# LabJunBMI/E3-invaraint-diffusion-model

Hardware: AMD Instinct MI355X
Metric: denoising-steps/sec (batched pocket graphs) (higher is better)
Workload: dtype f32 storage and accumulation, f16x3 products (fp32 grade); 1 GPU; structure_model sampling step, 256 x 256-residue pockets per GPU, 12+12 layers x 768, T=1000 schedule, encoder recomputed every step (as the reference); pockets_per_gpu=256, seq_len=256, parallelism=pocket-sharded x1, no collective

## Files before the change

e3-invaraint-diffusion-model_amd/bert.py:

```python
from dataclasses import dataclass

import os

import torch
from torch import nn

from . import ops
from .autograd import functional as F


@dataclass
class BertConfig:
    hidden_size: int = 768
    num_attention_heads: int = 12
    intermediate_size: int = 1024
    num_hidden_layers: int = 12
    max_position_embeddings: int = 64
    position_embedding_type: str = "relative_key"
    hidden_dropout_prob: float = 0.1
    attention_probs_dropout_prob: float = 0.1
    layer_norm_eps: float = 1e-12
    hidden_act: str = "gelu"
    use_cache: bool = False
    is_decoder: bool = False
# ... 172 lines not shown
def run_self_attention(att, x, mask, B, L, drop=(0.0, 0.0), layout=None):
    sa = att.self
    w, b = qkv_weights(sa)
    qkv = F.linear(x, w, b, absmax=ops.absmax_slot(sa, "qkv", x.device))
    relkey = sa.position_embedding_type == "relative_key"
    if layout is not None:
        H = att.num_heads * 64
        ctx = ops.attention_varlen(qkv[:, :H], qkv[:, H:2 * H], qkv[:, 2 * H:], layout, layout, att.num_heads,
                                   dist_emb=sa.distance_embedding.weight if relkey else None,
                                   max_pos=sa.max_position_embeddings)
        return _attention_output(att, ctx, x)
    ctx = F.attention(qkv, None, B, att.num_heads, L, L, key_mask=mask,
                      dist_emb=sa.distance_embedding.weight if relkey else None,
                      max_pos=sa.max_position_embeddings, drop_p=drop[1], row_keys=drop_keys(drop),
                      planes_for=_planes_for(att, x, drop))
    return _attention_output(att, ctx, x, drop[0], drop_keys(drop))


def project_cross_kv(att, enc):
    w, b = kv_weights(att.self)
    return F.linear(enc, w, b, absmax=torch.zeros(1, device=enc.device, dtype=torch.float32))


def run_cross_attention(att, x, kv, enc_mask, B, Lq, Lk, drop=(0.0, 0.0), layout=None, enc_layout=None):
    q = F.linear(x, att.self.query.weight, att.self.query.bias, absmax=ops.absmax_slot(att.self, "q", x.device))
    if layout is not None:
        H = att.num_heads * 64
        ctx = ops.attention_varlen(q, kv[:, :H], kv[:, H:], layout, enc_layout, att.num_heads)
        return _attention_output(att, ctx, x)
    ctx = F.attention(q, kv, B, att.num_heads, Lq, Lk, key_mask=enc_mask, drop_p=drop[1], row_keys=drop_keys(drop),
                      planes_for=_planes_for(att, x, drop))
    return _attention_output(att, ctx, x, drop[0], drop_keys(drop))


def run_layer(layer, x, mask, B, L, cross_kv=None, enc_mask=None, Lk=None, drop=(0.0, 0.0), layout=None,
              enc_layout=None):
    x = run_self_attention(layer.attention, x, mask, B, L, drop, layout=layout)
    if hasattr(layer, "crossattention"):
        if cross_kv is None:
            raise ValueError("decoder layer needs encoder states")
        x = run_cross_attention(layer.crossattention, x, cross_kv, enc_mask, B, L, Lk, drop, layout=layout,
                                enc_layout=enc_layout)
    inter = F.linear(x, layer.intermediate.dense.weight, layer.intermediate.dense.bias, ops.ACT_GELU,
                     planes_for=(layer.output.dense.weight, x) if drop[0] == 0 and drop[1] == 0 else None)
    return F.linear_residual_layernorm(inter, layer.output.dense.weight, layer.output.dense.bias, x,
                                       layer.output.LayerNorm.weight, layer.output.LayerNorm.bias, layer.eps, drop[0],
# ... 17 lines not shown
```

e3-invaraint-diffusion-model_amd/csrc/gemm_split.hip:

```cpp
#include <type_traits>

#include "e3d_common.h"

namespace {

typedef __bf16 bf16x8 __attribute__((ext_vector_type(8)));
typedef __bf16 bf16x4 __attribute__((ext_vector_type(4)));
typedef _Float16 f16x8 __attribute__((ext_vector_type(8)));
typedef _Float16 f16x4 __attribute__((ext_vector_type(4)));

template <typename E> struct Vec;
template <> struct Vec<__bf16> { typedef bf16x8 x8; typedef bf16x4 x4; };
template <> struct Vec<_Float16> { typedef f16x8 x8; typedef f16x4 x4; };
__device__ __forceinline__ f32x16 mma16(const bf16x8 a, const bf16x8 b, const f32x16 c) {
    return __builtin_amdgcn_mfma_f32_32x32x16_bf16(a, b, c, 0, 0, 0);
}
__device__ __forceinline__ f32x16 mma16(const f16x8 a, const f16x8 b, const f32x16 c) {
    return __builtin_amdgcn_mfma_f32_32x32x16_f16(a, b, c, 0, 0, 0);
}

struct Epi { float* absmax; float scale; int plan_m = 0; const int* run_if = nullptr; };

constexpr int BN = 128, BK = 32;
#ifdef GEMM_STAMPS
// ... 689 lines not shown
            const int col = col0 + wc * 64 + n * 32 + l31;
            const float bv = bias ? bias[col] : 0.f;
#pragma unroll
            for (int r = 0; r < 16; ++r) {
                const int row = row0 + wr * 128 + m * 32 + mfma32_row(r, half);
                float v = fmaf(acc[m][n][r], out_scale, bv);
                if (ACT == E3D_ACT_GELU) v = gelu_erf(v);
                if (ACT == E3D_ACT_SILU) v = silu(v);
                if (row < M) {
                    out[(int64_t)row * ldc + col] = v;
                    if (ACT == E3D_ACT_NONE && absmax) e3d_absmax_accum(amax, v);
                }
            }
        }
    }
    if (ACT == E3D_ACT_NONE && absmax) e3d_absmax_commit(amax, absmax, lane);
    STAMP_K(4);
#ifdef E3D_STAMPS
    asm volatile("s_waitcnt vmcnt(0)" ::: "memory");
    STAMP_K(5);
#endif
}

#ifdef E3D_NT_STORES
#define E3D_STORE_OUT(ptr, val) __builtin_nontemporal_store((val), (ptr))
#else
#define E3D_STORE_OUT(ptr, val) (*(ptr) = (val))
#endif

template <int ACT, typename E, bool PLANES = false>
__global__ __launch_bounds__(512, 2) void gemm_split256p_kernel(const float* __restrict__ A, int64_t lda,
                                                                 const float* __restrict__ W,
                                                                 const float* __restrict__ bias,
                                                                 float* __restrict__ out, int64_t ldc, int N, int K,
                                                                 int tiles_m, int tiles_n, float* __restrict__ absmax, float out_scale,
                                                                 const int* __restrict__ run_if) {
    if (run_if && *run_if == 0) return;
    extern __shared__ __attribute__((aligned(16))) unsigned char smem_raw[];
    constexpr int NS = 2, T_BYTES = BT * ROW64, BUF_BYTES = 2 * NS * T_BYTES;
    constexpr int NI = 8;
    const int total = tiles_m * tiles_n, nk = K / BK;
    const int tid = threadIdx.x, lane = tid & 63, wid = tid >> 6;
    const int wr = wid >> 2, wc = wid & 3;
    const int l31 = lane & 31, half = lane >> 5;

    unsigned goff[NI];
    int dst[NI];
#pragma unroll
    for (int i = 0; i < NI; ++i) {
        const int f = tid + 512 * (i & 3), r = f >> 3, kg = f & 7;
        goff[i] = (unsigned)(r * (i < 4 ? (int)lda : K) + kg * 4);
        dst[i] = (i < 4 ? 0 : NS * T_BYTES) + swz_off(r, kg >> 1) + (kg & 1) * 8;
    }

    int ld_tile = blockIdx.x, ld_k = 0;
    const float* ld_a;
    const float* ld_w;
    auto cursor_bases = [&]() {
        const int lid = xcd_remap(ld_tile, total);
        ld_a = A + (int64_t)(lid / tiles_n) * BT * lda + ld_k * BK;
        ld_w = W + (int64_t)(lid % tiles_n) * BT * K + ld_k * BK;
    };
    auto cursor_advance = [&]() {
        if (ld_k + 1 < nk) {
            ++ld_k;
            ld_a += BK;
            ld_w += BK;
        } else if (ld_tile + (int)gridDim.x < total) {
            ld_tile += gridDim.x;
            ld_k = 0;
            cursor_bases();
        }
    };
    f32x4 rg[NI];
    auto item_load = [&](int i) { rg[i] = *reinterpret_cast<const f32x4*>((i < 4 ? ld_a : ld_w) + goff[i]); };
    auto item_store = [&](int i, unsigned char* buf) {
        typename Vec<E>::x4 p[NS];
        split4<NS, E>(rg[i], p);
#pragma unroll
        for (int s = 0; s < NS; ++s) *reinterpret_cast<typename Vec<E>::x4*>(buf + s * T_BYTES + dst[i]) = p[s];
    };
    cursor_bases();
#pragma unroll
    for (int i = 0; i < NI; ++i) item_load(i);
    cursor_advance();
#pragma unroll
    for (int i = 0; i < NI; ++i) item_store(i, smem_raw);
#pragma unroll
    for (int i = 0; i < NI; ++i) item_load(i);
    cursor_advance();
    __syncthreads();

    int a_row[4], b_row[2];
#pragma unroll
    for (int m = 0; m < 4; ++m) a_row[m] = wr * 128 + m * 32 + l31;
#pragma unroll
    for (int n = 0; n < 2; ++n) b_row[n] = wc * 64 + n * 32 + l31;
    int cur = 0;
    unsigned amax = 0;

    for (int tile = blockIdx.x; tile < total; tile += gridDim.x) {
        f32x16 acc[4][2];
#pragma unroll
        for (int m = 0; m < 4; ++m)
#pragma unroll
            for (int n = 0; n < 2; ++n)
#pragma unroll
                for (int r = 0; r < 16; ++r) acc[m][n][r] = 0.f;
        for (int kt = 0; kt < nk; ++kt) {
            const unsigned char* base = smem_raw + cur * BUF_BYTES;
            unsigned char* next = smem_raw + (cur ^ 1) * BUF_BYTES;
#pragma unroll
            for (int ks = 0; ks < 2; ++ks) {
                typename Vec<E>::x8 fa[NS][4], fb[NS][2];
#pragma unroll
                for (int s = 0; s < NS; ++s) {
#pragma unroll
                    for (int n = 0; n < 2; ++n)
                        fb[s][n] = *reinterpret_cast<const typename Vec<E>::x8*>(base + (NS + s) * T_BYTES +
                                                                    swz_off(b_row[n], 2 * ks + half));
#pragma unroll
                    for (int m = 0; m < 4; ++m)
// ... 55 lines not shown
                        for (int j = 0; j < 4; ++j) {
                            float a = fmaf(acc[m][n][8 * kl + j], out_scale, bl[8 * kl + j]);
                            float c = fmaf(acc[m][n][8 * kl + 4 + j], out_scale, bl[8 * kl + 4 + j]);
                            if (ACT == E3D_ACT_GELU) { a = gelu_erf(a); c = gelu_erf(c); }
                            if (ACT == E3D_ACT_SILU) { a = silu(a); c = silu(c); }
                            if (ACT == E3D_ACT_NONE && absmax) { e3d_absmax_accum(amax, a); e3d_absmax_accum(amax, c); }
                            asm volatile("" : "+v"(a));
                            asm volatile("" : "+v"(c));
                            const auto sw = __builtin_amdgcn_permlane32_swap(__float_as_uint(a), __float_as_uint(c), false, false);
                            x0[j] = __uint_as_float(sw[0]);
                            x1[j] = __uint_as_float(sw[1]);
                        }
                        typename Vec<E>::x4 p0[2], p1[2];
                        split4<2, E>(x0, p0);
                        split4<2, E>(x1, p1);
                        typedef typename Vec<E>::x8 X8;
                        *reinterpret_cast<X8*>(o + kl * 2048) = __builtin_shufflevector(p0[0], p1[0], 0, 1, 2, 3, 4, 5, 6, 7);
                        *reinterpret_cast<X8*>(o + kl * 2048 + 1024) = __builtin_shufflevector(p0[1], p1[1], 0, 1, 2, 3, 4, 5, 6, 7);
                    }
                }
            }
            continue;
        }
        const int lid = xcd_remap(tile, total);
        const int row0 = (lid / tiles_n) * BT, col0 = (lid % tiles_n) * BT;
#pragma unroll
        for (int m = 0; m < 4; ++m) {
#pragma unroll
            for (int n = 0; n < 2; ++n) {
                const int col = col0 + wc * 64 + n * 32 + l31;
                const float bv = bias ? bias[col] : 0.f;
                float* o = out + (int64_t)(row0 + wr * 128 + m * 32 + 4 * half) * ldc + col;
#pragma unroll
                for (int r = 0; r < 16; ++r) {
                    float v = fmaf(acc[m][n][r], out_scale, bv);
                    if (ACT == E3D_ACT_GELU) v = gelu_erf(v);
                    if (ACT == E3D_ACT_SILU) v = silu(v);
                    E3D_STORE_OUT(&o[(int64_t)((r & 3) + 8 * (r >> 2)) * ldc], v);
                    if (ACT == E3D_ACT_NONE && absmax) e3d_absmax_accum(amax, v);
                }
            }
        }
    }
    if (ACT == E3D_ACT_NONE && absmax) e3d_absmax_commit(amax, absmax, lane);
}

template <int ACT, typename E, bool PLANES = false>
int launch256p(const float* A, int64_t lda, const float* W, const float* bias, float* out, int64_t ldc, int M, int N,
               int K, Epi epi, hipStream_t s) {
    const int tiles_m = M / BT, tiles_n = N / BT;
    constexpr size_t lds = 2 * 2 * 2 * BT * ROW64;
    static std::atomic<uint64_t> lds_ok{0};
    const int n_cu = e3d_cu_count();
    const int total = tiles_m * tiles_n;
    e3d_allow_lds(lds_ok, gemm_split256p_kernel<ACT, E, PLANES>, lds);
    hipLaunchKernelGGL((gemm_split256p_kernel<ACT, E, PLANES>), dim3(total < n_cu ? total : n_cu), dim3(512), lds, s, A, lda, W, bias, out,
                       ldc, N, K, tiles_m, tiles_n, epi.absmax, epi.scale, epi.run_if);
    return e3d_launch_status(PLANES ? "e3d_gemm_bias_act_planes_split (persistent 256x256)" : "e3d_gemm_f32_split (persistent 256x256)");
}

int g_general_form = -1;
int g_tile_pref = -1;

template <int NS, int ACT, int WR, int WC, int NBUF, bool PIPE, typename E>
int launch256(const float* A, int64_t lda, const float* W, const float* bias, float* out, int64_t ldc, int M, int N,
              int K, Epi epi, hipStream_t s) {
    constexpr int TM = WR * 128, TN = WC * 64;
    const int tiles_m = (M + TM - 1) / TM, tiles_n = N / TN;
    const size_t lds = (size_t)NBUF * NS * (TM + TN) * ROW64;
    static std::atomic<uint64_t> lds_ok{0};
    e3d_allow_lds(lds_ok, gemm_split256_kernel<NS, ACT, WR, WC, NBUF, PIPE, E>, lds);
    hipLaunchKernelGGL((gemm_split256_kernel<NS, ACT, WR, WC, NBUF, PIPE, E>), dim3(tiles_m * tiles_n), dim3(WR * WC * 64), lds, s,
                       A, lda, W, bias, out, ldc, M, N, K, tiles_m, tiles_n, epi.absmax, epi.scale, epi.run_if);
    return e3d_launch_status("e3d_gemm_f32_split (128x64 wave tiles)");
}

template <int NS, int ACT, bool A_KMAJ, bool B_KMAJ, int WM, int WN, typename E, int TN = 2, bool TR = false>
int launch_general(const float* A, int64_t lda, const float* B, int64_t ldb, const float* bias, float* out, int64_t ldc,
                   int M, int N, int K, Epi epi, hipStream_t s);

int p_min() {
    static int v = 0;
    if (!v) {
        const char* e = getenv("E3D_GEMM_P_MIN");
        v = e ? atoi(e) : 160;
    }
    return v;
}

bool persistent_ok(int M, int Mp, int N, int K, int64_t lda, int64_t ldb, int k_min = 2 * BK) {
    if (g_tile_pref < 0) {
        const char* e = getenv("E3D_GEMM_TILE");
        g_tile_pref = e ? atoi(e) : 4;
    }
    const int64_t n_tiles = (int64_t)(Mp / BT) * (N / BT);
    return N % BT == 0 && M % BT == 0 && Mp % BT == 0 && ldb == K && g_tile_pref >= 4 && K >= k_min && lda < (1 << 22) &&
           (g_tile_pref >= 5 || n_tiles >= p_min() || (n_tiles >= 96 && N >= 6 * BT && !getenv("E3D_GEMM_P_MIN")));
}

template <int NS, int ACT, bool A_KMAJ, bool B_KMAJ, typename E>
int launch(const float* A, int64_t lda, const float* B, int64_t ldb, const float* bias, float* out, int64_t ldc,
           int M, int N, int K, Epi epi, hipStream_t s) {
    if (g_tile_pref < 0) {
        const char* e = getenv("E3D_GEMM_TILE");
        g_tile_pref = e ? atoi(e) : 4;
    }
    const int Mp = epi.plan_m > 0 ? epi.plan_m : M;
    if constexpr (!A_KMAJ && !B_KMAJ) {
        if constexpr (NS == 2) {
            if (persistent_ok(M, Mp, N, K, lda, ldb))
                return launch256p<ACT, E>(A, lda, B, bias, out, ldc, M, N, K, epi, s);
            if (N % BT == 0 && ldb == K && g_tile_pref >= 3 && (int64_t)((Mp + BT - 1) / BT) * (N / BT) >= 256)
                return launch256<NS, ACT, 2, 4, 2, true, E>(A, lda, B, bias, out, ldc, M, N, K, epi, s);
        }
        if constexpr (NS == 1) {
            if (N % BT == 0 && ldb == K && g_tile_pref >= 3 && (int64_t)((Mp + BT - 1) / BT) * (N / BT) >= 160)
                return launch256<NS, ACT, 2, 4, 2, true, E>(A, lda, B, bias, out, ldc, M, N, K, epi, s);
        }
        if (N % BT == 0 && ldb == K && g_tile_pref >= 1 &&
            (int64_t)((Mp + BT - 1) / BT) * (N / BT) >= 256)
            return launch256<NS, ACT, 2, 4, (NS <= 2 ? 2 : 1), false, E>(A, lda, B, bias, out, ldc, M, N, K, epi, s);
    }
    if (g_general_form < 0) {
        const char* e = getenv("E3D_GEMM_FORM");
        g_general_form = e ? atoi(e) : 0;
    }
    int form = g_general_form;
    if (form != 1 && form != 2 && form != 3 && form != 4) {
        const int64_t g256 = (int64_t)((Mp + 255) / 256) * ((N + 127) / 128), g128 = (int64_t)((Mp + 127) / 128) * ((N + 127) / 128);
        const int64_t cus = e3d_cu_count();
        if (NS == 3) form = g256 < 128 && !A_KMAJ && !B_KMAJ ? 2 : 1;
        else if (A_KMAJ && B_KMAJ) form = 1;
        else if (A_KMAJ) form = g128 <= cus ? 2 : (g256 <= cus ? 1 : (45 * ((g128 + 2 * cus - 1) / (2 * cus)) < 37 * ((g256 + cus - 1) / cus) ? 2 : 1));
        else form = 25 * ((g128 + cus - 1) / cus) <= 38 * ((g256 + cus - 1) / cus) ? 3 : 1;
// ... 76 lines not shown
    if (a_kmaj && b_kmaj) return launch<NS, E3D_ACT_NONE, true, true, __bf16>(A, lda, B, ldb, bias, out, ldc, M, N, K, Epi{nullptr, epi.scale}, s);
    return launch<NS, E3D_ACT_NONE, true, false, __bf16>(A, lda, B, ldb, bias, out, ldc, M, N, K, epi, s);
}

}

#ifdef GEMM_STAMPS
extern "C" int e3d_debug_gemm_stamps(long long* t) { return (int)hipMemcpyFromSymbol(t, HIP_SYMBOL(gemm_stamps), sizeof(long long) * 2 * 64 * 8); }
#endif

#ifdef E3D_STAMPS
extern "C" int e3d_debug_read_stamps(long long* host_out) {
    return (int)hipMemcpyFromSymbol(host_out, HIP_SYMBOL(e3d_stamps), sizeof(long long) * 2 * 32 * 8);
}
#endif

extern "C" int e3d_gemm_kernel_select(int pref) {
    if (g_tile_pref < 0) {
        const char* e = getenv("E3D_GEMM_TILE");
        g_tile_pref = e ? atoi(e) : 4;
    }
    const int prev = g_tile_pref;
    if (pref >= 0) g_tile_pref = pref;
    return prev;
}

extern "C" int e3d_gemm_general_select(int form) {
    if (g_general_form < 0) {
        const char* e = getenv("E3D_GEMM_FORM");
        g_general_form = e ? atoi(e) : 0;
    }
    const int prev = g_general_form;
    if (form >= 0) g_general_form = form;
    return prev;
}

static int gemm_split_general(const float* A, int64_t lda, int a_kmajor, const float* B, int64_t ldb, int b_kmajor,
                              const float* bias, float* out, int64_t ldc, int M, int N, int K, int act, int terms,
                              float* absmax, float out_scale, void* stream, int plan_m = 0, const int* run_if = nullptr) {
    const Epi epi{absmax, out_scale, plan_m, run_if};
    E3D_REQUIRE(plan_m >= 0 && (!(a_kmajor || b_kmajor) || (plan_m == 0 && !run_if)),
                "gemm_split: plan_m / run_if exist for the forward (K-contiguous) layout (plan_m=%d)", plan_m);
    E3D_REQUIRE(out_scale == 1.0f || !(a_kmajor && b_kmajor), "gemm_split: out_scale is not available for the split-K layout");
    E3D_REQUIRE(A && B && out, "gemm_split: null pointer");
    E3D_REQUIRE(M > 0 && N > 0 && K > 0, "gemm_split: bad shape M=%d N=%d K=%d", M, N, K);
    E3D_REQUIRE(terms == E3D_TERMS_BF16 || terms == 3 || terms == 6 || terms == E3D_TERMS_F16X3,
// ... 145 lines not shown
    return (terms == 3 || terms == E3D_TERMS_F16X3) && (act == E3D_ACT_NONE || act == E3D_ACT_GELU) && M > 0 && N > 0 && K > 0 &&
           K % BK == 0 && lda >= K && lda % 4 == 0 && persistent_ok(M, M, N, K, lda, K, BK);
}

extern "C" int e3d_gemm_bias_act_planes_split(const float* A, int64_t lda, const float* W, const float* bias, void* out_planes,
                                              int M, int N, int K, int act, int terms, float* out_absmax, float out_scale,
                                              void* stream) {
    E3D_REQUIRE(A && W && out_planes, "gemm_split (planes): null pointer");
    E3D_REQUIRE(e3d_gemm_planes_supported(M, N, K, lda, act, terms),
                "gemm_split (planes): this launch does not take the persistent kernel (M=%d N=%d K=%d act=%d terms=%d)", M, N, K, act, terms);
    E3D_REQUIRE(((uintptr_t)A % 16) == 0 && ((uintptr_t)W % 16) == 0 && ((uintptr_t)bias % 16) == 0 && ((uintptr_t)out_planes % 16) == 0,
                "gemm_split (planes): A, W, bias and the planes must be 16-byte aligned");
    E3D_REQUIRE(!out_absmax || act == E3D_ACT_NONE, "gemm_split (planes): out_absmax exists for act = none");
    const Epi epi{out_absmax, out_scale, 0, nullptr};
    hipStream_t s = (hipStream_t)stream;
    float* out = reinterpret_cast<float*>(out_planes);
    if (terms == 3) {
        if (act == E3D_ACT_GELU) return launch256p<E3D_ACT_GELU, __bf16, true>(A, lda, W, bias, out, N, M, N, K, epi, s);
        return launch256p<E3D_ACT_NONE, __bf16, true>(A, lda, W, bias, out, N, M, N, K, epi, s);
    }
    if (act == E3D_ACT_GELU) return launch256p<E3D_ACT_GELU, _Float16, true>(A, lda, W, bias, out, N, M, N, K, epi, s);
    return launch256p<E3D_ACT_NONE, _Float16, true>(A, lda, W, bias, out, N, M, N, K, epi, s);
}
```

e3-invaraint-diffusion-model_amd/hip.py:

```python
import ctypes
import os
from ctypes import c_char_p, c_float, c_int, c_int64, c_uint32, c_uint64, c_void_p

_HERE = os.path.dirname(os.path.abspath(__file__))
LIB_PATH = os.environ.get("E3D_HIP_LIB", os.path.join(_HERE, "libe3d_hip.so"))
ABI_VERSION = 5

_P = c_void_p
_VIEW = [_P, c_int64, c_int64]
_QKV = 3 * _VIEW + [_P, c_int, _P]
_SHAPE = 4 * [c_int]
_ATTN_FWD = _QKV + [_P, _P] + _SHAPE
_ATTN_BWD = _QKV + 3 * [_P] + 3 * _VIEW + [_P, _P] + _SHAPE
_STREAM = [_P]
_DROP = [c_float, c_uint64]
_DROP_KEYED = [c_float, c_uint32, _P]
_BOUNDS = [_P, c_int, _P, _P, _P]
_SIGNATURES = {
    "e3d_abi_version": (c_int, []),
    "e3d_last_error": (c_char_p, []),
    "e3d_gemm_bias_act_f32": (c_int, [_P, c_int64, _P, _P, _P, c_int64, c_int, c_int, c_int, c_int, _P]),
    "e3d_gemm_bias_act_f32_split": (c_int, [_P, c_int64, _P, _P, _P, c_int64, c_int, c_int, c_int, c_int, c_int, _P]),
    "e3d_gemm_bias_act_f32_split_ex": (c_int, [_P, c_int64, _P, _P, _P, c_int64, c_int, c_int, c_int, c_int, c_int, _P, c_float, _P]),
    "e3d_gemm_bias_act_f32_split_gated": (c_int, [_P, c_int64, _P, _P, _P, c_int64, c_int, c_int, c_int, c_int, c_int, _P, c_float,
                                                  c_int, _P, _P]),
    "e3d_absmax_f32": (c_int, [_P, c_int64, _P, _P]),
    "e3d_relkey_attn_fwd": (c_int, _ATTN_FWD + _STREAM),
    "e3d_relkey_attn_fwd_split": (c_int, _ATTN_FWD + [c_int] + _STREAM),
    "e3d_gemm_skinny_workspace_bytes": (c_int64, [c_int, c_int, c_int]),
    "e3d_gemm_skinny_f32_split": (c_int, [_P, c_int64, _P, _P, _P, c_int64, c_int, c_int, c_int, c_int, c_int, _P, c_int64, _P]),
    "e3d_gemm_skinny_f32_split_ex": (c_int, [_P, c_int64, _P, _P, _P, c_int64, c_int, c_int, c_int, c_int, c_int, _P, c_int64, _P, c_float, _P]),
    "e3d_gemm_skinny_plan_select": (None, [c_int, c_int]),
    "e3d_gemm_skinny_residual_layernorm_f32_split": (c_int, [_P, c_int64, _P, _P, _P, _P, _P, c_float, _P, c_int, c_int, c_int,
                                                     c_int, _P, c_int64, _P]),
    "e3d_gemm_skinny_residual_layernorm_f32_split_ex": (c_int, [_P, c_int64, _P, _P, _P, _P, _P, c_float, _P, c_int, c_int, c_int,
                                                        c_int, _P, c_int64, c_float, _P]),
    "e3d_attn_skip_padded_tiles": (c_int, [c_int]),
    "e3d_gemm_kernel_select": (c_int, [c_int]),
    "e3d_gemm_general_select": (c_int, [c_int]),
    "e3d_attn_rescale_tau": (c_float, [c_float]),
    "e3d_residual_layernorm_fwd": (c_int, [_P, _P, _P, _P, c_float, _P, _P, c_int, c_int, _P]),
    "e3d_adaln_gate_fwd": (c_int, [_P, _P, _P, c_int, c_int, _P, c_int, c_int, _P]),
    "e3d_embed_layernorm_fwd": (c_int, [_P, c_int, _P, _P, _P, _P, c_float, _P, c_int, _P, _P, c_int, c_int, _P]),
    "e3d_adaln_gate_indexed_fwd": (c_int, [_P, _P, _P, _P, c_int, _P, c_int, _P, c_int, c_int, _P]),
    "e3d_classify_onehot_rows": (c_int, [_P, c_int, _P, _P, c_int, _P]),
    "e3d_embed_layernorm_fwd_ex": (c_int, [_P, c_int, _P, _P, _P, _P, c_float, _P, c_int, _P, _P, c_int, c_int, _P, _P]),
    "e3d_nerf_backbone": (c_int, [_P, _P, _P, c_int, c_int, c_int, _P]),
    "e3d_gemm_f32_split_general": (c_int, [_P, c_int64, c_int, _P, c_int64, c_int, _P, _P, c_int64, c_int, c_int,
                                           c_int, c_int, c_int, _P]),
    "e3d_transpose_grouped_f32": (c_int, [_P, _P, c_int, c_int, c_int, c_int64, c_int64, _P]),
    "e3d_gemm_wgrad_grouped_f32_split": (c_int, [_P, _P, _P, _P, c_uint64, c_int, c_int64, c_int64, c_int, c_int, c_int, c_int, _P]),
    "e3d_residual_layernorm_drop_fwd": (c_int, [_P, _P, _P, _P, c_float, _P, _P, c_int, c_int, c_float, c_uint64, _P]),
    "e3d_layernorm_bwd_drop": (c_int, [_P, _P, _P, c_float, _P, _P, _P, _P, c_int, c_int, c_float, c_uint64, _P]),
    "e3d_weight_planes_bytes": (c_int64, [c_int, c_int]),
    "e3d_weight_planes_f32_split": (c_int, [_P, c_int, c_int, c_int, _P, _P]),
    "e3d_gemm_residual_layernorm_supported": (c_int, [c_int, c_int, c_int, c_int64]),
    "e3d_gemm_residual_layernorm_f32_split": (c_int, [_P, c_int64, _P, _P, _P, c_int64, _P, _P, c_float, _P, c_int64,
                                                      c_int, c_int, c_int, c_int, c_float, _P]),
    "e3d_activation_planes_bytes": (c_int64, [c_int, c_int]),
    "e3d_activation_planes_f32_split": (c_int, [_P, c_int64, c_int, c_int, c_int, _P, _P]),
    "e3d_gemm_residual_layernorm_planes_split": (c_int, [_P, _P, _P, _P, c_int64, _P, _P, c_float, _P, c_int64,
                                                         c_int, c_int, c_int, c_int, c_float, _P]),
    "e3d_gemm_planes_supported": (c_int, [c_int, c_int, c_int, c_int64, c_int, c_int]),
    "e3d_gemm_bias_act_planes_split": (c_int, [_P, c_int64, _P, _P, _P, c_int, c_int, c_int, c_int, c_int, _P, c_float, _P]),
    "e3d_attn_planes_supported": (c_int, [c_int64, c_int64, c_int64, c_int, c_int, c_int, c_int]),
    "e3d_relkey_attn_fwd_split_planes": (c_int, _QKV + [_P] + _SHAPE + [c_int] + _BOUNDS + _STREAM),
    "e3d_gemm_wgrad_ragged_f32_split": (c_int, [_P, _P, _P, _P, _P, _P, _P, _P, c_uint64, c_int, c_int, c_int, _P]),
    "e3d_relkey_attn_bwd_workspace_floats": (c_int64, [c_int, c_int, c_int, c_int, c_int]),
    "e3d_relkey_attn_bwd": (c_int, _ATTN_BWD + _STREAM),
    "e3d_dropout_f32": (c_int, [_P, c_float, c_uint64, _P, c_int64, _P]),
    "e3d_relkey_attn_fwd_split_drop": (c_int, _ATTN_FWD + [c_int] + _DROP + _STREAM),
    "e3d_relkey_attn_fwd_split_ex": (c_int, _ATTN_FWD + [c_int] + _DROP + _BOUNDS + _STREAM),
    "e3d_attn_scratch_bytes": (c_int64, [c_int]),
    "e3d_ddpm_step_wrap_table": (c_int, [_P, _P, _P, _P, _P, c_int, _P, c_int64, _P]),
    "e3d_relkey_attn_bwd_drop": (c_int, _ATTN_BWD + _DROP + _STREAM),
    "e3d_relkey_attn_bwd_ex": (c_int, _ATTN_BWD + [c_int] + _DROP + _STREAM),
    "e3d_attn_dropout_mask": (c_int, [c_int, c_int, c_int, c_int, c_float, c_uint64, _P, _P]),
    "e3d_layernorm_bwd": (c_int, [_P, _P, _P, c_float, _P, _P, _P, c_int, c_int, _P]),
    "e3d_layernorm_bwd_workspace_floats": (c_int64, [c_int, c_int]),
    "e3d_layernorm_bwd_ws": (c_int, [_P, _P, _P, c_float, _P, _P, _P, _P, c_int, c_int, c_float, c_uint64, _P, c_int64, _P]),
    "e3d_adaln_gate_bwd": (c_int, [_P, _P, _P, c_int, c_int, _P, _P, c_int, c_int, _P]),
    "e3d_act_fwd": (c_int, [_P, c_int, _P, c_int64, _P]),
    "e3d_act_bwd": (c_int, [_P, _P, c_int, _P, c_int64, _P]),
    "e3d_colsum": (c_int, [_P, c_int64, _P, c_int, c_int, _P]),
    "e3d_group_sum": (c_int, [_P, c_int, _P, c_int, c_int, _P]),
    "e3d_small_k_wgrad": (c_int, [_P, _P, _P, _P, c_int, c_int, c_int, c_int, _P]),
    "e3d_head_linear_bwd_dx": (c_int, [_P, _P, _P, c_int, c_int, c_int, _P]),
# ... 83 lines not shown
```

e3-invaraint-diffusion-model_amd/ops.py:

```python
import contextlib
import math
import os
import warnings

import torch

from . import hip, keyed

ACT_NONE, ACT_GELU, ACT_SILU = 0, 1, 2


def _stream():
    return torch.cuda.current_stream().cuda_stream


TRACE = None


_ROCTX = None


def _roctx():
    global _ROCTX
    if _ROCTX is None:
# ... 219 lines not shown
        _chk(run_if, "gemm.run_if", torch.int32)
        plan_m = M if plan_m is None else plan_m
        if not gemm_is_tiled(plan_m, mode):
            raise ValueError(f"gemm: plan_m / run_if exist on the tiled split kernels only (plan_m={plan_m}, mode={mode or GEMM_MODE})")
        with _timed("gemm" if run_if is None else "gemm_gated", (M, N, K, act)):
            hip.check(hip.lib().e3d_gemm_bias_act_f32_split_gated(
                _p(a), a.stride(0), _p(weight), _p(bias), _p(out), out.stride(0), M, N, K, act, terms, _p(absmax), scale,
                plan_m, _p(run_if), _stream()), "e3d_gemm_bias_act_f32_split_gated")
        return out
    with _timed("gemm", (M, N, K, act)):
        if _skinny_ok(terms, M, N, K, a) and out.stride(0) % 4 == 0 and M <= min(SKINNY_MAX_M, SKINNY_GEMM_MAX_M):
            ws = _skinny_workspace(a.device, M, N, K)
            hip.check(hip.lib().e3d_gemm_skinny_f32_split_ex(_p(a), a.stride(0), _p(weight), _p(bias), _p(out), out.stride(0),
                                                             M, N, K, act, terms, _p(ws), ws.numel(), _p(absmax), scale, _stream()),
                      "e3d_gemm_skinny_f32_split_ex")
        elif terms == 0:
            hip.check(hip.lib().e3d_gemm_bias_act_f32(_p(a), a.stride(0), _p(weight), _p(bias), _p(out),
                                                      out.stride(0), M, N, K, act, _stream()), "e3d_gemm_bias_act_f32")
        else:
            hip.check(hip.lib().e3d_gemm_bias_act_f32_split_ex(
                _p(a), a.stride(0), _p(weight), _p(bias), _p(out), out.stride(0), M, N, K, act, terms, _p(absmax), scale,
                _stream()), "e3d_gemm_bias_act_f32_split_ex")
    return out


class arithmetic:

    def __init__(self, mode, respect_env=True):
        self.gemm = os.environ.get("E3D_GEMM_MODE", mode) if respect_env else mode
        self.attn = os.environ.get("E3D_ATTN_MODE", self.gemm) if respect_env else mode

    def __enter__(self):
        self.prev = (set_gemm_mode(self.gemm), set_attn_mode(self.attn))
        return self

    def __exit__(self, *exc):
        set_gemm_mode(self.prev[0])
        set_attn_mode(self.prev[1])


ATTN_MODE = os.environ.get("E3D_ATTN_MODE", GEMM_MODE)
if ATTN_MODE == "bf16":
    ATTN_MODE = "bf16x3"
if ATTN_MODE not in GEMM_MODES:
    raise ValueError(f"E3D_ATTN_MODE must be one of {sorted(GEMM_MODES)}, got {ATTN_MODE!r}")

# ... 879 lines not shown
```

e3-invaraint-diffusion-model_amd/structure_model/model.py:

```python
import functools
from typing import List

import torch
from torch import nn

from .. import bert, keyed, ops
from ..blocks import (BertEmbeddings, GaussianFourierProjection, KeyedDropoutSwitch, Predictor, SELayer, drop_row_keys,
                      flat2d, onehot_modulation, require_gpu)
from ..training import adamw
import os

from .utils import elementwise_form, radian_l1_loss, radian_smooth_l1_loss

MASKED_LOSS = os.environ.get("E3D_MASKED_LOSS", "1") == "1"


class ReceptorCache:

    def __init__(self, encoder_states, cross_kv, mask, B, L, layout=None):
        self.encoder_states, self.cross_kv, self.mask, self.B, self.L = encoder_states, cross_kv, mask, B, L
        self.layout = layout


class ConditionalBertForDiffusionBase(nn.Module):
# ... 3 lines not shown
        self.decoder_config = decoder_config
        self.receptor_seq_emb = BertEmbeddings(20, encoder_config)
        self.receptor_angle_emb = BertEmbeddings(feature_size, encoder_config)
        self.receptor_emb = SELayer(encoder_config)
        self.encoder = bert.BertEncoder(encoder_config)
        self.ligand_angle_emb = BertEmbeddings(feature_size, decoder_config)
        self.timestep_projector = GaussianFourierProjection(decoder_config.hidden_size)
        self.timestep_emb = SELayer(decoder_config)
        self.decoder = bert.BertEncoder(decoder_config)
        self.angles_predictor = Predictor(decoder_config.hidden_size, feature_size)

    def encode_receptor(self, receptor_seq, receptor_angles, receptor_attention_masks,
                        project_cross_kv=True, layout=None) -> ReceptorCache:
        require_gpu(receptor_seq, receptor_angles, receptor_attention_masks)
        B, L = receptor_angles.shape[:2]
        ops.reset_absmax(receptor_angles.device)
        if layout is not None:
            ang = self.receptor_angle_emb.run(flat2d(layout.pack(receptor_angles)))
            seq2d = flat2d(layout.pack(receptor_seq))
            mod = onehot_modulation(self.receptor_emb, self.receptor_seq_emb, seq2d)
            seq = self.receptor_seq_emb.run(seq2d) if mod is None else None
            x = self.receptor_emb.run(ang, seq, None, 1, layout.rows, mod=mod, layout=layout)
            x = bert.run_encoder(self.encoder, x, None, 1, layout.rows, layout=layout)
            kv = [bert.project_cross_kv(layer.crossattention, x) for layer in self.decoder.layer] if project_cross_kv else None
            return ReceptorCache(x, kv, None, B, L, layout=layout)
        mask = receptor_attention_masks.contiguous().float()
        rk = drop_row_keys(keyed.DROP_POCKET, L)
        ang = self.receptor_angle_emb.run(flat2d(receptor_angles), row_keys=rk)
        seq2d = flat2d(receptor_seq)
        mod = onehot_modulation(self.receptor_emb, self.receptor_seq_emb, seq2d)
        seq = self.receptor_seq_emb.run(seq2d, row_keys=rk) if mod is None else None
        x = self.receptor_emb.run(ang, seq, mask, B, L, mod=mod, row_keys=rk)
        x = bert.run_encoder(self.encoder, x, mask, B, L, row_keys=rk)
        kv = None
        if project_cross_kv:
            kv = [bert.project_cross_kv(layer.crossattention, x) for layer in self.decoder.layer]
        return ReceptorCache(x, kv, mask, B, L)

    def timestep_modulation(self, timesteps):
        temb = self.timestep_projector(timesteps.reshape(-1)).contiguous()
        return self.timestep_emb.modulation(temb)

    def decode(self, timestep, noised_ligand_angles, ligand_attention_masks, receptor: ReceptorCache, mod=None,
               layout=None):
        if layout is not None:
            return self._decode_packed(timestep, noised_ligand_angles, receptor, mod, layout)
        require_gpu(timestep, noised_ligand_angles, ligand_attention_masks)
        B, L = noised_ligand_angles.shape[:2]
        mask = ligand_attention_masks.contiguous().float()
        lk = drop_row_keys(keyed.DROP_LIGAND, L)
        x = self.ligand_angle_emb.run(flat2d(noised_ligand_angles), row_keys=lk)
        if mod is None:
            mod = self.timestep_modulation(timestep.squeeze(dim=-1))
        x = self.timestep_emb.run(x, None, mask, B, L, mod=mod, row_keys=lk)
        x = bert.run_encoder(self.decoder, x, mask, B, L, enc=receptor.encoder_states,
                             enc_mask=receptor.mask, Lk=receptor.L, cross_kv=receptor.cross_kv, row_keys=lk)
        return self.angles_predictor.run(x).view(B, L, -1)

    def _decode_packed(self, timestep, x_packed, receptor, mod, layout):
# ... 112 lines not shown
```

include/e3d_hip.h:

```cpp
#ifndef E3D_HIP_H
#define E3D_HIP_H

#include <stdint.h>

#ifdef __cplusplus
extern "C" {
#endif

#define E3D_ABI_VERSION 5

#define E3D_TERMS_BF16 1
#define E3D_TERMS_BF16X3 3
#define E3D_TERMS_BF16X6 6
#define E3D_TERMS_F16X3 19

#define E3D_ACT_NONE 0
#define E3D_ACT_GELU 1
#define E3D_ACT_SILU 2

int e3d_abi_version(void);
const char* e3d_last_error(void);

int e3d_gemm_bias_act_f32(const float* A, int64_t lda, const float* W, const float* bias,
                          float* out, int64_t ldc, int M, int N, int K, int act, void* stream);
// ... 23 lines not shown
                              float* out, float* lse, int B, int nh, int Lq, int Lk, int terms,
                              void* stream);

int64_t e3d_gemm_skinny_workspace_bytes(int M, int N, int K);
int e3d_gemm_skinny_f32_split(const float* A, int64_t lda, const float* W, const float* bias, float* out,
                              int64_t ldc, int M, int N, int K, int act, int terms, void* workspace,
                              int64_t workspace_bytes, void* stream);
int e3d_gemm_skinny_f32_split_ex(const float* A, int64_t lda, const float* W, const float* bias, float* out,
                                 int64_t ldc, int M, int N, int K, int act, int terms, void* workspace,
                                 int64_t workspace_bytes, float* out_absmax, float out_scale, void* stream);
void e3d_gemm_skinny_plan_select(int waves_per_cu_x2, int min_k_slice);
int e3d_gemm_skinny_residual_layernorm_f32_split(const float* A, int64_t lda, const float* W, const float* bias,
                                                 const float* residual, const float* gamma, const float* beta, float eps,
                                                 float* out, int M, int H, int K, int terms, void* workspace,
                                                 int64_t workspace_bytes, void* stream);
int e3d_gemm_skinny_residual_layernorm_f32_split_ex(const float* A, int64_t lda, const float* W, const float* bias,
                                                    const float* residual, const float* gamma, const float* beta,
                                                    float eps, float* out, int M, int H, int K, int terms,
                                                    void* workspace, int64_t workspace_bytes, float out_scale,
                                                    void* stream);

int e3d_gemm_kernel_select(int pref);
int e3d_gemm_general_select(int form);

float e3d_attn_rescale_tau(float tau);

int e3d_attn_skip_padded_tiles(int enable);

int e3d_residual_layernorm_fwd(const float* x, const float* residual, const float* gamma,
                               const float* beta, float eps, float* s_out, float* out, int M,
                               int H, void* stream);

int e3d_adaln_gate_fwd(const float* x, const float* y, const float* mod, int branch,
                       int rows_per_cond, float* out, int M, int H, void* stream);

int e3d_adaln_gate_indexed_fwd(const float* x, const float* y, const int* idx, const float* table, int table_rows,
                               const float* mod, int branch, float* out, int M, int H, void* stream);

int e3d_classify_onehot_rows(const float* x, int F, int* idx, int* flag, int M, void* stream);

int e3d_embed_layernorm_fwd(const float* x, int F, const float* W, const float* b,
                            const float* gamma, const float* beta, float eps,
                            const float* post_add, int rows_per_add, float* z_out, float* out,
                            int M, int H, void* stream);
int e3d_embed_layernorm_fwd_ex(const float* x, int F, const float* W, const float* b,
                               const float* gamma, const float* beta, float eps,
// ... 180 lines not shown
                                    float* s_out, float* out, int M, int H, float drop_p, uint64_t drop_seed, void* stream);
int e3d_layernorm_bwd_drop(const float* dy, const float* s, const float* gamma, float eps, float* ds, float* ds_dropped,
                           float* dgamma, float* dbeta, int M, int H, float drop_p, uint64_t drop_seed, void* stream);
int64_t e3d_layernorm_bwd_workspace_floats(int M, int H);
int e3d_layernorm_bwd_ws(const float* dy, const float* s, const float* gamma, float eps, float* ds, float* ds_dropped,
                         float* dgamma, float* dbeta, int M, int H, float drop_p, uint64_t drop_seed, float* workspace,
                         int64_t workspace_floats, void* stream);

int64_t e3d_weight_planes_bytes(int N, int K);
int e3d_weight_planes_f32_split(const float* W, int N, int K, int terms, void* planes, void* stream);
int e3d_gemm_residual_layernorm_supported(int M, int N, int K, int64_t lda);
int e3d_gemm_residual_layernorm_f32_split(const float* A, int64_t lda, const void* w_planes, const float* bias,
                                          const float* residual, int64_t ldr, const float* gamma, const float* beta, float eps,
                                          float* out, int64_t ldo, int M, int N, int K, int terms, float out_scale, void* stream);

int64_t e3d_activation_planes_bytes(int M, int K);
int e3d_activation_planes_f32_split(const float* X, int64_t ldx, int M, int K, int terms, void* planes, void* stream);
int e3d_gemm_residual_layernorm_planes_split(const void* a_planes, const void* w_planes, const float* bias,
                                             const float* residual, int64_t ldr, const float* gamma, const float* beta, float eps,
                                             float* out, int64_t ldo, int M, int N, int K, int terms, float out_scale, void* stream);
int e3d_gemm_planes_supported(int M, int N, int K, int64_t lda, int act, int terms);
int e3d_gemm_bias_act_planes_split(const float* A, int64_t lda, const float* W, const float* bias, void* out_planes,
                                   int M, int N, int K, int act, int terms, float* out_absmax, float out_scale, void* stream);
int e3d_attn_planes_supported(int64_t k_rs, int64_t v_bs, int64_t v_rs, int Lq, int Lk, int terms, int have_scratch);
int e3d_relkey_attn_fwd_split_planes(const float* q, int64_t q_bs, int64_t q_rs, const float* k, int64_t k_bs,
                                     int64_t k_rs, const float* v, int64_t v_bs, int64_t v_rs,
                                     const float* dist_emb, int P, const float* key_mask, void* out_planes,
                                     int B, int nh, int Lq, int Lk, int terms, void* e_scratch, int e_scratch_ready,
                                     const float* q_absmax, const float* k_absmax, float* e_absmax, void* stream);

int e3d_adamw_step_dyn(float* const* params, const float* const* grads, float* const* exp_avg, float* const* exp_avg_sq,
                       const int64_t* numel, const int* chunk_tensor, const int64_t* chunk_first, int n_chunks,
                       const float* norm_and_clip, const float* lr_and_step, float beta1, float beta2, float eps,
                       float weight_decay, void* stream);
int e3d_adamw_step_dev(float* const* params, const float* const* grads, float* const* exp_avg, float* const* exp_avg_sq,
                       const int64_t* numel, const int* chunk_tensor, const int64_t* chunk_first, int n_chunks,
                       const float* norm_and_clip, const float* hyper, void* stream);
int e3d_dropout_set_epoch_ptr(const uint64_t* device_word);
int e3d_optim_chunk_elems(void);
int e3d_grad_global_norm(const float* const* grads, const int64_t* numel, const int* chunk_tensor, const int64_t* chunk_first,
                         int n_chunks, float max_norm, float* partial, float* norm_and_clip, void* stream);
int e3d_adamw_step(float* const* params, const float* const* grads, float* const* exp_avg, float* const* exp_avg_sq,
                   const int64_t* numel, const int* chunk_tensor, const int64_t* chunk_first, int n_chunks,
                   const float* norm_and_clip, float lr, float beta1, float beta2, float eps, float weight_decay, int step,
                   void* stream);

// ... 60 lines not shown
```

Before: 4118 pocket-steps/s.

## Group the decoder cross-attention KV projections into one shared-A persistent GEMM launch

Adds a grouped mode to the persistent 256x256 split GEMM kernel, so that all 12 decoder layers' cross-attention K/V projections of the same encoder output run as a single launch over the concatenated tile space, with per-group weight, bias, output and absmax pointers. This removes 11 separate kernel launches and their tail waves on each step. It also adds nontemporal streaming stores for large fp32 GEMM outputs, by default for outputs of 512 MB and up and always on in the grouped path, so that the large KV outputs do not pollute the cache. The risk is that streaming stores could hurt if the KV tensors are read again soon, since the cross-attention consumes them within the same step.

```diff
diff --git a/e3-invaraint-diffusion-model_amd/bert.py b/e3-invaraint-diffusion-model_amd/bert.py
--- a/e3-invaraint-diffusion-model_amd/bert.py
+++ b/e3-invaraint-diffusion-model_amd/bert.py
@@ -218,6 +218,28 @@
     return F.linear(enc, w, b, absmax=torch.zeros(1, device=enc.device, dtype=torch.float32))
 
 
+CROSS_KV_GROUPED = os.environ.get("E3D_CROSS_KV_GROUPED", "1") != "0"
+
+
+def project_cross_kv_all(decoder_layers, enc, layout=None):
+    atts = [layer.crossattention for layer in decoder_layers]
+    if not CROSS_KV_GROUPED or layout is not None or torch.is_grad_enabled() or not ops.gemm_is_tiled(enc.shape[0]):
+        return [project_cross_kv(att, enc) for att in atts]
+    packs = [kv_weights(att.self) for att in atts]
+    out = []
+    for i in range(0, len(packs), ops.SHARED_A_MAX):
+        ws, bs = zip(*packs[i:i + ops.SHARED_A_MAX])
+        if not ops.gemm_shared_a_ok(enc, ws, bs):
+            out += [project_cross_kv(att, enc) for att in atts[i:i + ops.SHARED_A_MAX]]
+            continue
+        bounds = list(torch.zeros(len(ws), device=enc.device, dtype=torch.float32).split(1))
+        kvs = ops.gemm_shared_a(enc, ws, bs, absmax=bounds)
+        for kv, bound in zip(kvs, bounds):
+            kv._e3d_absmax = bound
+        out += kvs
+    return out
+
+
 def run_cross_attention(att, x, kv, enc_mask, B, Lq, Lk, drop=(0.0, 0.0), layout=None, enc_layout=None):
     q = F.linear(x, att.self.query.weight, att.self.query.bias, absmax=ops.absmax_slot(att.self, "q", x.device))
     if layout is not None:
diff --git a/e3-invaraint-diffusion-model_amd/csrc/gemm_split.hip b/e3-invaraint-diffusion-model_amd/csrc/gemm_split.hip
--- a/e3-invaraint-diffusion-model_amd/csrc/gemm_split.hip
+++ b/e3-invaraint-diffusion-model_amd/csrc/gemm_split.hip
@@ -735,24 +735,34 @@
 #endif
 }
 
-#ifdef E3D_NT_STORES
-#define E3D_STORE_OUT(ptr, val) __builtin_nontemporal_store((val), (ptr))
-#else
-#define E3D_STORE_OUT(ptr, val) (*(ptr) = (val))
-#endif
-
-template <int ACT, typename E, bool PLANES = false>
+constexpr int SHARED_A_MAX = 16;
+struct SharedAGroups {
+    const float* W[SHARED_A_MAX];
+    const float* bias[SHARED_A_MAX];
+    float* out[SHARED_A_MAX];
+    float* absmax[SHARED_A_MAX];
+    float scale[SHARED_A_MAX];
+    int count;
+};
+struct NoGroups {};
+
+template <int ACT, typename E, bool PLANES = false, bool GROUPED = false, bool STREAM = false>
 __global__ __launch_bounds__(512, 2) void gemm_split256p_kernel(const float* __restrict__ A, int64_t lda,
                                                                  const float* __restrict__ W,
                                                                  const float* __restrict__ bias,
                                                                  float* __restrict__ out, int64_t ldc, int N, int K,
                                                                  int tiles_m, int tiles_n, float* __restrict__ absmax, float out_scale,
-                                                                 const int* __restrict__ run_if) {
+                                                                 const int* __restrict__ run_if,
+                                                                 const std::conditional_t<GROUPED, SharedAGroups, NoGroups> grp) {
+    static_assert(!GROUPED || (ACT == E3D_ACT_NONE && !PLANES), "the grouped form writes fp32 rows without activation");
+    static_assert(!STREAM || !PLANES, "streaming stores exist for the fp32 row output");
     if (run_if && *run_if == 0) return;
     extern __shared__ __attribute__((aligned(16))) unsigned char smem_raw[];
     constexpr int NS = 2, T_BYTES = BT * ROW64, BUF_BYTES = 2 * NS * T_BYTES;
     constexpr int NI = 8;
-    const int total = tiles_m * tiles_n, nk = K / BK;
+    const int per = tiles_m * tiles_n, nk = K / BK;
+    int total = per;
+    if constexpr (GROUPED) total = per * grp.count;
     const int tid = threadIdx.x, lane = tid & 63, wid = tid >> 6;
     const int wr = wid >> 2, wc = wid & 3;
     const int l31 = lane & 31, half = lane >> 5;
@@ -770,9 +780,15 @@
     const float* ld_a;
     const float* ld_w;
     auto cursor_bases = [&]() {
-        const int lid = xcd_remap(ld_tile, total);
+        int lid = xcd_remap(ld_tile, total);
+        const float* w = W;
+        if constexpr (GROUPED) {
+            const int g = __builtin_amdgcn_readfirstlane(lid / per);
+            lid -= g * per;
+            w = grp.W[g];
+        }
         ld_a = A + (int64_t)(lid / tiles_n) * BT * lda + ld_k * BK;
-        ld_w = W + (int64_t)(lid % tiles_n) * BT * K + ld_k * BK;
+        ld_w = w + (int64_t)(lid % tiles_n) * BT * K + ld_k * BK;
     };
     auto cursor_advance = [&]() {
         if (ld_k + 1 < nk) {
@@ -811,6 +827,7 @@
     for (int n = 0; n < 2; ++n) b_row[n] = wc * 64 + n * 32 + l31;
     int cur = 0;
     unsigned amax = 0;
+    [[maybe_unused]] int cur_g = -1;
 
     for (int tile = blockIdx.x; tile < total; tile += gridDim.x) {
         f32x16 acc[4][2];
@@ -912,7 +929,20 @@
             }
             continue;
         }
-        const int lid = xcd_remap(tile, total);
+        int lid = xcd_remap(tile, total);
+        if constexpr (GROUPED) {
+            const int g = __builtin_amdgcn_readfirstlane(lid / per);
+            lid -= g * per;
+            if (g != cur_g) {
+                if (cur_g >= 0 && absmax) e3d_absmax_commit(amax, absmax, lane);
+                amax = 0;
+                cur_g = g;
+            }
+            bias = grp.bias[g];
+            out = grp.out[g];
+            absmax = grp.absmax[g];
+            out_scale = grp.scale[g];
+        }
         const int row0 = (lid / tiles_n) * BT, col0 = (lid % tiles_n) * BT;
 #pragma unroll
         for (int m = 0; m < 4; ++m) {
@@ -926,7 +956,9 @@
                     float v = fmaf(acc[m][n][r], out_scale, bv);
                     if (ACT == E3D_ACT_GELU) v = gelu_erf(v);
                     if (ACT == E3D_ACT_SILU) v = silu(v);
-                    E3D_STORE_OUT(&o[(int64_t)((r & 3) + 8 * (r >> 2)) * ldc], v);
+                    float* const dst_v = &o[(int64_t)((r & 3) + 8 * (r >> 2)) * ldc];
+                    if constexpr (STREAM) __builtin_nontemporal_store(v, dst_v);
+                    else *dst_v = v;
                     if (ACT == E3D_ACT_NONE && absmax) e3d_absmax_accum(amax, v);
                 }
             }
@@ -935,7 +967,7 @@
     if (ACT == E3D_ACT_NONE && absmax) e3d_absmax_commit(amax, absmax, lane);
 }
 
-template <int ACT, typename E, bool PLANES = false>
+template <int ACT, typename E, bool PLANES = false, bool STREAM = false>
 int launch256p(const float* A, int64_t lda, const float* W, const float* bias, float* out, int64_t ldc, int M, int N,
                int K, Epi epi, hipStream_t s) {
     const int tiles_m = M / BT, tiles_n = N / BT;
@@ -943,10 +975,24 @@
     static std::atomic<uint64_t> lds_ok{0};
     const int n_cu = e3d_cu_count();
     const int total = tiles_m * tiles_n;
-    e3d_allow_lds(lds_ok, gemm_split256p_kernel<ACT, E, PLANES>, lds);
-    hipLaunchKernelGGL((gemm_split256p_kernel<ACT, E, PLANES>), dim3(total < n_cu ? total : n_cu), dim3(512), lds, s, A, lda, W, bias, out,
-                       ldc, N, K, tiles_m, tiles_n, epi.absmax, epi.scale, epi.run_if);
+    e3d_allow_lds(lds_ok, gemm_split256p_kernel<ACT, E, PLANES, false, STREAM>, lds);
+    hipLaunchKernelGGL((gemm_split256p_kernel<ACT, E, PLANES, false, STREAM>), dim3(total < n_cu ? total : n_cu), dim3(512), lds, s, A,
+                       lda, W, bias, out, ldc, N, K, tiles_m, tiles_n, epi.absmax, epi.scale, epi.run_if, NoGroups{});
     return e3d_launch_status(PLANES ? "e3d_gemm_bias_act_planes_split (persistent 256x256)" : "e3d_gemm_f32_split (persistent 256x256)");
+}
+
+template <typename E, bool STREAM>
+int launch256p_shared_a(const float* A, int64_t lda, const SharedAGroups& g, int M, int N, int K, hipStream_t s) {
+    const int tiles_m = M / BT, tiles_n = N / BT;
+    constexpr size_t lds = 2 * 2 * 2 * BT * ROW64;
+    static std::atomic<uint64_t> lds_ok{0};
+    const int n_cu = e3d_cu_count();
+    const int total = tiles_m * tiles_n * g.count;
+    e3d_allow_lds(lds_ok, gemm_split256p_kernel<E3D_ACT_NONE, E, false, true, STREAM>, lds);
+    hipLaunchKernelGGL((gemm_split256p_kernel<E3D_ACT_NONE, E, false, true, STREAM>), dim3(total < n_cu ? total : n_cu), dim3(512), lds,
+                       s, A, lda, (const float*)nullptr, (const float*)nullptr, (float*)nullptr, (int64_t)N, N, K, tiles_m, tiles_n,
+                       (float*)nullptr, 1.0f, (const int*)nullptr, g);
+    return e3d_launch_status("e3d_gemm_bias_f32_split_shared_a (persistent 256x256)");
 }
 
 int g_general_form = -1;
@@ -978,6 +1024,16 @@
     return v;
 }
 
+int64_t g_stream_min_bytes = -1;
+int64_t stream_min_bytes() {
+    if (g_stream_min_bytes < 0) {
+        const char* e = getenv("E3D_GEMM_STREAM_MIN_MB");
+        g_stream_min_bytes = e ? (int64_t)atoll(e) << 20 : (int64_t)512 << 20;
+        if (g_stream_min_bytes < 0) g_stream_min_bytes = 0;
+    }
+    return g_stream_min_bytes;
+}
+
 bool persistent_ok(int M, int Mp, int N, int K, int64_t lda, int64_t ldb, int k_min = 2 * BK) {
     if (g_tile_pref < 0) {
         const char* e = getenv("E3D_GEMM_TILE");
@@ -998,8 +1054,14 @@
     const int Mp = epi.plan_m > 0 ? epi.plan_m : M;
     if constexpr (!A_KMAJ && !B_KMAJ) {
         if constexpr (NS == 2) {
-            if (persistent_ok(M, Mp, N, K, lda, ldb))
+            if (persistent_ok(M, Mp, N, K, lda, ldb)) {
+                if constexpr (ACT == E3D_ACT_NONE) {
+                    const int64_t min_bytes = stream_min_bytes();
+                    if (min_bytes > 0 && (int64_t)M * N * 4 >= min_bytes)
+                        return launch256p<ACT, E, false, true>(A, lda, B, bias, out, ldc, M, N, K, epi, s);
+                }
                 return launch256p<ACT, E>(A, lda, B, bias, out, ldc, M, N, K, epi, s);
+            }
             if (N % BT == 0 && ldb == K && g_tile_pref >= 3 && (int64_t)((Mp + BT - 1) / BT) * (N / BT) >= 256)
                 return launch256<NS, ACT, 2, 4, 2, true, E>(A, lda, B, bias, out, ldc, M, N, K, epi, s);
         }
@@ -1122,6 +1184,12 @@
     }
     const int prev = g_tile_pref;
     if (pref >= 0) g_tile_pref = pref;
+    return prev;
+}
+
+extern "C" int64_t e3d_gemm_stream_min_bytes(int64_t bytes) {
+    const int64_t prev = stream_min_bytes();
+    if (bytes >= 0) g_stream_min_bytes = bytes;
     return prev;
 }
 
@@ -1313,3 +1381,38 @@
     if (act == E3D_ACT_GELU) return launch256p<E3D_ACT_GELU, _Float16, true>(A, lda, W, bias, out, N, M, N, K, epi, s);
     return launch256p<E3D_ACT_NONE, _Float16, true>(A, lda, W, bias, out, N, M, N, K, epi, s);
 }
+
+extern "C" int e3d_gemm_shared_a_supported(int M, int N, int K, int count, int64_t lda, int terms) {
+    return (terms == 3 || terms == E3D_TERMS_F16X3) && count >= 1 && count <= SHARED_A_MAX && M > 0 && N > 0 && K > 0 &&
+           N % BT == 0 && K % BK == 0 && lda >= K && lda % 4 == 0 && (int64_t)count * N < (1ll << 30) &&
+           (int64_t)(M / BT) * (N / BT) * count < (1ll << 30) && persistent_ok(M, M, count * N, K, lda, K, BK);
+}
+
+extern "C" int e3d_gemm_bias_f32_split_shared_a(const float* A, int64_t lda, const float* const* W, const float* const* bias,
+                                                float* const* out, float* const* out_absmax, const float* out_scale, int count,
+                                                int M, int N, int K, int terms, int stream_stores, void* stream) {
+    E3D_REQUIRE(A && W && out, "gemm_split (shared A): null pointer");
+    E3D_REQUIRE(e3d_gemm_shared_a_supported(M, N, K, count, lda, terms),
+                "gemm_split (shared A): this launch does not take the persistent kernel (M=%d N=%d K=%d count=%d lda=%lld terms=%d)",
+                M, N, K, count, (long long)lda, terms);
+    E3D_REQUIRE(((uintptr_t)A % 16) == 0, "gemm_split (shared A): A must be 16-byte aligned");
+    SharedAGroups g;
+    for (int p = 0; p < SHARED_A_MAX; ++p) {
+        const int q = p < count ? p : 0;
+        E3D_REQUIRE(W[q] && out[q], "gemm_split (shared A): null pointer in problem %d", q);
+        E3D_REQUIRE(((uintptr_t)W[q] % 16) == 0 && ((uintptr_t)out[q] % 16) == 0 && (!bias || ((uintptr_t)bias[q] % 16) == 0) &&
+                    (!out_absmax || ((uintptr_t)out_absmax[q] % 4) == 0),
+                    "gemm_split (shared A): W, bias and out of problem %d must be 16-byte aligned", q);
+        g.W[p] = W[q]; g.bias[p] = bias ? bias[q] : nullptr; g.out[p] = out[q];
+        g.absmax[p] = out_absmax ? out_absmax[q] : nullptr;
+        g.scale[p] = out_scale ? out_scale[q] : 1.0f;
+    }
+    g.count = count;
+    hipStream_t s = (hipStream_t)stream;
+    if (terms == 3) {
+        if (stream_stores) return launch256p_shared_a<__bf16, true>(A, lda, g, M, N, K, s);
+        return launch256p_shared_a<__bf16, false>(A, lda, g, M, N, K, s);
+    }
+    if (stream_stores) return launch256p_shared_a<_Float16, true>(A, lda, g, M, N, K, s);
+    return launch256p_shared_a<_Float16, false>(A, lda, g, M, N, K, s);
+}
diff --git a/e3-invaraint-diffusion-model_amd/hip.py b/e3-invaraint-diffusion-model_amd/hip.py
--- a/e3-invaraint-diffusion-model_amd/hip.py
+++ b/e3-invaraint-diffusion-model_amd/hip.py
@@ -38,6 +38,7 @@
     "e3d_attn_skip_padded_tiles": (c_int, [c_int]),
     "e3d_gemm_kernel_select": (c_int, [c_int]),
     "e3d_gemm_general_select": (c_int, [c_int]),
+    "e3d_gemm_stream_min_bytes": (c_int64, [c_int64]),
     "e3d_attn_rescale_tau": (c_float, [c_float]),
     "e3d_residual_layernorm_fwd": (c_int, [_P, _P, _P, _P, c_float, _P, _P, c_int, c_int, _P]),
     "e3d_adaln_gate_fwd": (c_int, [_P, _P, _P, c_int, c_int, _P, c_int, c_int, _P]),
@@ -63,6 +64,8 @@
                                                          c_int, c_int, c_int, c_int, c_float, _P]),
     "e3d_gemm_planes_supported": (c_int, [c_int, c_int, c_int, c_int64, c_int, c_int]),
     "e3d_gemm_bias_act_planes_split": (c_int, [_P, c_int64, _P, _P, _P, c_int, c_int, c_int, c_int, c_int, _P, c_float, _P]),
+    "e3d_gemm_shared_a_supported": (c_int, [c_int, c_int, c_int, c_int, c_int64, c_int]),
+    "e3d_gemm_bias_f32_split_shared_a": (c_int, [_P, c_int64, _P, _P, _P, _P, _P, c_int, c_int, c_int, c_int, c_int, c_int, _P]),
     "e3d_attn_planes_supported": (c_int, [c_int64, c_int64, c_int64, c_int, c_int, c_int, c_int]),
     "e3d_relkey_attn_fwd_split_planes": (c_int, _QKV + [_P] + _SHAPE + [c_int] + _BOUNDS + _STREAM),
     "e3d_gemm_wgrad_ragged_f32_split": (c_int, [_P, _P, _P, _P, _P, _P, _P, _P, c_uint64, c_int, c_int, c_int, _P]),
diff --git a/e3-invaraint-diffusion-model_amd/ops.py b/e3-invaraint-diffusion-model_amd/ops.py
--- a/e3-invaraint-diffusion-model_amd/ops.py
+++ b/e3-invaraint-diffusion-model_amd/ops.py
@@ -1,4 +1,5 @@
 import contextlib
+import ctypes
 import math
 import os
 import warnings
@@ -265,6 +266,51 @@
                 _p(a), a.stride(0), _p(weight), _p(bias), _p(out), out.stride(0), M, N, K, act, terms, _p(absmax), scale,
                 _stream()), "e3d_gemm_bias_act_f32_split_ex")
     return out
+
+
+SHARED_A_MAX = 16
+SHARED_A_STREAM = os.environ.get("E3D_SHARED_A_STREAM", "1") != "0"
+
+
+def gemm_shared_a_ok(a, weights, biases, mode=None):
+    terms = GEMM_MODES[GEMM_MODE if mode is None else mode]
+    if terms not in (3, 19) or not 1 <= len(weights) <= SHARED_A_MAX or len(biases) != len(weights):
+        return False
+    if not (a.is_cuda and a.dtype == torch.float32 and a.dim() == 2 and a.stride(1) == 1 and a.data_ptr() % 16 == 0):
+        return False
+    M, K = a.shape
+    N = weights[0].shape[0]
+    for w, b in zip(weights, biases):
+        if not (w.is_cuda and w.dtype == torch.float32 and w.is_contiguous() and tuple(w.shape) == (N, K)):
+            return False
+        if b is not None and not (b.is_cuda and b.dtype == torch.float32 and b.is_contiguous() and b.numel() == N
+                                  and b.data_ptr() % 16 == 0):
+            return False
+    ok = hip.lib().e3d_gemm_shared_a_supported
+    return bool(K >= 64 and ok(M, N, K, 1, a.stride(0), terms) and ok(M, N, K, len(weights), a.stride(0), terms))
+
+
+def gemm_shared_a(a, weights, biases, absmax=None, mode=None, stream_stores=None):
+    G = len(weights)
+    M, K = a.shape
+    N = weights[0].shape[0]
+    terms = GEMM_MODES[GEMM_MODE if mode is None else mode]
+    absmax = [None] * G if absmax is None else list(absmax)
+    for t in absmax:
+        _chk(t, "gemm_shared_a.absmax")
+    scales = [1.0] * G
+    if terms == 19:
+        weights, scales = zip(*(f16_weight(w) for w in weights))
+    for w in weights:
+        assert w.data_ptr() % 16 == 0
+    outs = list(torch.empty((G, M, N), device=a.device, dtype=torch.float32).unbind(0))
+    ptrs = lambda ts: (ctypes.c_void_p * G)(*[_p(t) for t in ts])
+    stream_stores = SHARED_A_STREAM if stream_stores is None else stream_stores
+    with _timed("gemm", (M, G * N, K, ACT_NONE)):
+        hip.check(hip.lib().e3d_gemm_bias_f32_split_shared_a(
+            _p(a), a.stride(0), ptrs(weights), ptrs(biases), ptrs(outs), ptrs(absmax), (ctypes.c_float * G)(*scales), G,
+            M, N, K, terms, int(bool(stream_stores)), _stream()), "e3d_gemm_bias_f32_split_shared_a")
+    return outs
 
 
 class arithmetic:
diff --git a/e3-invaraint-diffusion-model_amd/structure_model/model.py b/e3-invaraint-diffusion-model_amd/structure_model/model.py
--- a/e3-invaraint-diffusion-model_amd/structure_model/model.py
+++ b/e3-invaraint-diffusion-model_amd/structure_model/model.py
@@ -49,7 +49,7 @@
             seq = self.receptor_seq_emb.run(seq2d) if mod is None else None
             x = self.receptor_emb.run(ang, seq, None, 1, layout.rows, mod=mod, layout=layout)
             x = bert.run_encoder(self.encoder, x, None, 1, layout.rows, layout=layout)
-            kv = [bert.project_cross_kv(layer.crossattention, x) for layer in self.decoder.layer] if project_cross_kv else None
+            kv = bert.project_cross_kv_all(self.decoder.layer, x, layout=layout) if project_cross_kv else None
             return ReceptorCache(x, kv, None, B, L, layout=layout)
         mask = receptor_attention_masks.contiguous().float()
         rk = drop_row_keys(keyed.DROP_POCKET, L)
@@ -61,7 +61,7 @@
         x = bert.run_encoder(self.encoder, x, mask, B, L, row_keys=rk)
         kv = None
         if project_cross_kv:
-            kv = [bert.project_cross_kv(layer.crossattention, x) for layer in self.decoder.layer]
+            kv = bert.project_cross_kv_all(self.decoder.layer, x)
         return ReceptorCache(x, kv, mask, B, L)
 
     def timestep_modulation(self, timesteps):
diff --git a/include/e3d_hip.h b/include/e3d_hip.h
--- a/include/e3d_hip.h
+++ b/include/e3d_hip.h
@@ -69,6 +69,7 @@
 
 int e3d_gemm_kernel_select(int pref);
 int e3d_gemm_general_select(int form);
+int64_t e3d_gemm_stream_min_bytes(int64_t bytes);
 
 float e3d_attn_rescale_tau(float tau);
 
@@ -295,6 +296,10 @@
 int e3d_gemm_planes_supported(int M, int N, int K, int64_t lda, int act, int terms);
 int e3d_gemm_bias_act_planes_split(const float* A, int64_t lda, const float* W, const float* bias, void* out_planes,
                                    int M, int N, int K, int act, int terms, float* out_absmax, float out_scale, void* stream);
+int e3d_gemm_shared_a_supported(int M, int N, int K, int count, int64_t lda, int terms);
+int e3d_gemm_bias_f32_split_shared_a(const float* A, int64_t lda, const float* const* W, const float* const* bias,
+                                     float* const* out, float* const* out_absmax, const float* out_scale, int count, int M,
+                                     int N, int K, int terms, int stream_stores, void* stream);
 int e3d_attn_planes_supported(int64_t k_rs, int64_t v_bs, int64_t v_rs, int Lq, int Lk, int terms, int have_scratch);
 int e3d_relkey_attn_fwd_split_planes(const float* q, int64_t q_bs, int64_t q_rs, const float* k, int64_t k_bs,
                                      int64_t k_rs, const float* v, int64_t v_bs, int64_t v_rs,
```

After: 4149 pocket-steps/s (median of 6 runs). Within noise of the previous version (+0.8%).
